# bdwsq1996/Effi-MVS-plus

Hardware: AMD Instinct MI355X
Metric: ref-views/sec (cost-volume hot path: warp + cost volume + 3-D regularisation + cascaded GRU refinement) (higher is better)
Workload: dtype f32 (3x3 MFMA convs: products as 3 bf16 partial products hi*hi+hi*lo+lo*hi, f32 accumulate; all else f32); 1 GPU; cfg3: DTU-shaped 1600x1184, N=5 views (S=4 sources), 3-stage cascade ndepths=48,8,8, GRU iters 3,3,3, seeded-random weights, features of the stock FPN resident in HBM; parallelism=single GPU, views_in_flight=3, arithmetic=split

## Files before the change

### effi_mvs_plus_amd/csrc/api.hip

```cpp
#include "common.hpp"
#include "launch_form.hpp"
#include <cstdlib>
#include <cstring>
#include <mutex>

extern "C" int effi_version(void) { return 200; }

extern "C" const char* effi_error_string(int code) {
    switch (code) {
        case EFFI_OK: return "ok";
        case EFFI_ERR_BADARG: return "bad argument (null pointer, non-positive size, or inconsistent shapes)";
        case EFFI_ERR_UNSUPPORTED: return "shape / channel count not instantiated in this build";
        case EFFI_ERR_LAUNCH: return "kernel launch failed (hipPeekAtLastError)";
        case EFFI_ERR_WORKSPACE: return "no workspace registered for the current device (effi_set_workspace)";
        default: return "unknown error code";
    }
}

static const void* g_workspace[EFFI_MAX_DEVICES];

extern "C" long effi_workspace_bytes(void) { return 256; }

extern "C" int effi_set_workspace(int device, void* workspace, long bytes) {
    if (device < 0 || device >= EFFI_MAX_DEVICES) return EFFI_ERR_BADARG;
// ... 4 lines not shown

extern "C" const void* effi_get_workspace(int device) {
    if (device < 0 || device >= EFFI_MAX_DEVICES) return nullptr;
    return __atomic_load_n(&g_workspace[device], __ATOMIC_ACQUIRE);
}

const float* effi_zero_page() {
    int dev = -1;
    if (hipGetDevice(&dev) != hipSuccess) return nullptr;
    return (const float*)effi_get_workspace(dev);
}

namespace {
const char* const kOptName[EFFI_OPT_COUNT] = {"warp_lds_kb", "dyn_form", "dyn_setup_exact", "dyn_xchg", "pixnet_mfma", "force_mr", "mr4_min",
                                              "mr4_nt2_max", "mr2_min", "wide_tiles", "roll_mr", "roll_zt", "roll_rp", "deconv_mr", "sr_waves", "enc_gen_mr3", "c3_lean", "dyn_win",
                                              "roll_slide"};
long g_opt[EFFI_OPT_COUNT];
std::once_flag g_opt_once;
void load_options() {
    for (int i = 0; i < EFFI_OPT_COUNT; ++i) {
        char env[64] = "EFFI_";
        size_t n = strlen(env);
        for (const char* c = kOptName[i]; *c && n + 1 < sizeof(env); ++c) env[n++] = (*c >= 'a' && *c <= 'z') ? (char)(*c - 32) : *c;
        env[n] = 0;
        const char* v = getenv(env);
        g_opt[i] = (v && *v) ? atol(v) : EFFI_OPT_UNSET;
    }
}
int find_option(const char* name) {
    if (!name) return -1;
    for (int i = 0; i < EFFI_OPT_COUNT; ++i)
// ... 28 lines not shown
    const EffiFormOpts o = effi_form_opts();
    EffiForm f;
    switch (launcher) {
        case EFFI_LF_X3: f = effi_pick_x3(nt, h, w, zb ? planes : 1, zb, sr, o); break;
        case EFFI_LF_X3_BATCH: f = effi_pick_x3_batch(nt, h, w, count, o); break;
        case EFFI_LF_X3_ZB_BATCH: f = effi_pick_x3_zb_batch(nt, h, w, (long)planes * count, o); break;
        case EFFI_LF_X3_PAIR: f = effi_pick_x3_pair(nt, h, w, sr, o); break;
        case EFFI_LF_CONV2D: f = effi_pick_generic(k1 ? 1 : 3, h, w, count); break;
        case EFFI_LF_PLANES3D: f = effi_pick_planes(h, w, (long)planes * count, s2 ? 2 : 4); break;
        case EFFI_LF_K5S2: f = effi_pick_planes(h, w, count, 2); break;
        case EFFI_LF_S2_X3: f = effi_pick_s2_x3(h, w, nt == 1 ? 1 : (nt + 1) / 2, (long)planes * count); break;
        case EFFI_LF_ROLL: f = effi_pick_roll((flags & EFFI_LF_FLAG_OCT2) ? 2 : 1, nt, cout, h, w, planes, count, o); break;
        case EFFI_LF_DECONV_X3: f = effi_pick_deconv_x3(cout, h, w, planes, count, o); break;
        case EFFI_LF_C3_PLANES: f = effi_pick_c3_planes(h, w, planes, count); break;
        case EFFI_LF_DECONV_K3: f = effi_pick_deconv_k3(cout, h, w, planes, count); break;
        default: return EFFI_ERR_BADARG;
    }
    form[0] = f.rows, form[1] = f.cols, form[2] = f.waves, form[3] = f.planes, form[4] = f.variant;
    return EFFI_OK;
}

namespace {
__global__ __launch_bounds__(256) void lds_poison_kernel(unsigned pattern, unsigned* sink) {
    __shared__ unsigned buf[16 * 1024];
    for (int i = threadIdx.x; i < 16 * 1024; i += 256) buf[i] = pattern;
    __syncthreads();
    if (buf[(threadIdx.x * 61) & 16383] != pattern) sink[0] = 1;
}
}

// ... 67 lines not shown
```

### effi_mvs_plus_amd/csrc/common.hpp

```cpp
#pragma once
#include <hip/hip_runtime.h>
#include "../../include/effi_mvs_hip.h"

#define EFFI_LAUNCH_CHECK()                                   \
    do {                                                      \
        if (hipPeekAtLastError() != hipSuccess) return EFFI_ERR_LAUNCH; \
    } while (0)

const float* effi_zero_page();

enum EffiOption {
    EFFI_OPT_WARP_LDS_KB,
    EFFI_OPT_DYN_FORM,
    EFFI_OPT_DYN_SETUP_EXACT,
    EFFI_OPT_DYN_XCHG,
    EFFI_OPT_PIXNET_MFMA,
    EFFI_OPT_FORCE_MR,
    EFFI_OPT_MR4_MIN, EFFI_OPT_MR4_NT2_MAX, EFFI_OPT_MR2_MIN,
    EFFI_OPT_WIDE_TILES,
    EFFI_OPT_ROLL_MR, EFFI_OPT_ROLL_ZT, EFFI_OPT_ROLL_RP,
    EFFI_OPT_DECONV_MR,
    EFFI_OPT_SR_WAVES,
    EFFI_OPT_ENC_GEN_MR3,
    EFFI_OPT_C3_LEAN,
    EFFI_OPT_DYN_WIN,
    EFFI_OPT_ROLL_SLIDE,
    EFFI_OPT_COUNT
};
constexpr long EFFI_OPT_UNSET = -0x7fffffffL;
long effi_option(int id);

static inline hipStream_t effi_s(effi_stream_t s) {
    (void)hipGetLastError();
    return reinterpret_cast<hipStream_t>(s);
}
static inline int effi_cdiv(long a, long b) { return (int)((a + b - 1) / b); }

struct EffiPtrList {
    const float* p[EFFI_MAX_VIEWS + 1];
    const float* const* tbl;
};
// ... 387 lines not shown
```

### effi_mvs_plus_amd/csrc/conv2d_x3.hpp

```cpp
#pragma once
#include "common.hpp"
#include "launch_form.hpp"
#include <type_traits>

#ifdef EFFI_BF16_ONLY
#define EFFI_FN(name) name##_bf16
#else
#define EFFI_FN(name) name
#endif

#ifndef EFFI_ABL
#define EFFI_ABL 0
#endif
#ifndef EFFI_PIPE_FRAGS
#define EFFI_PIPE_FRAGS 0
#endif

#ifndef EFFI_EPI_BATCH
#define EFFI_EPI_BATCH 1
#endif
#ifndef EFFI_EPI_EARLY_MAX
#define EFFI_EPI_EARLY_MAX 16
#endif
#ifndef EFFI_B_EARLY
// ... 23 lines not shown
    const float* aux1;
    const float* disp_range;
    int n_range;
    float* out0;
    float* out1;
    long cstride;
    long ostride;
    int zcount;
    int zin;
    int hin, win;
    const float* zeros;
    const float* xptr0;
    int sr_hp, sr_wp;
    unsigned short* out_sr;
    int aux_q4;
};

struct ConvBatch {
    int n_img;
    long src[EFFI_MAX_SRC];
    long aux0;
    long out0;
};

__device__ __forceinline__ Conv2dArgs conv_batch_image(Conv2dArgs a, const ConvBatch& b, int img) {
#pragma unroll
    for (int i = 0; i < EFFI_MAX_SRC; ++i) a.src[i] += (long)img * b.src[i];
    a.aux0 += (long)img * b.aux0;
    a.out0 += (long)img * b.out0;
    return a;
}

struct EncGenArgs {
    const float* inv_depth; const float* disp_range; int n_range; const float* interval;
    const float* cur_vol; long cds, cps; int Dcur;
    const float* reg_vol; long rds, rps; int Dreg;
    const float* dmin; const float* dmax; long range_ps;
    const float* w_c1; const float* b_c1;
    const float* w_d1; const float* b_d1;
    int hd;
    int off32;
};

__device__ __forceinline__ float apply_act(float v, int act) {
// ... 126 lines not shown

__device__ __forceinline__ void split_octet(const f32x4 (&pa)[8], int px, bf16x8& hi, bf16x8& lo) {
#pragma unroll
    for (int e = 0; e < 8; e += 2) {
        const f32x2 x = {pa[e][px], pa[e + 1][px]};
        const bf16x2 h2 = __builtin_convertvector(x, bf16x2);
        const f32x2 hf = __builtin_convertvector(h2, f32x2);
        const bf16x2 l2 = __builtin_convertvector(x - hf, bf16x2);
        hi[e] = h2[0];
        hi[e + 1] = h2[1];
        lo[e] = l2[0];
        lo[e + 1] = l2[1];
    }
}

template <int NT, int MR, int EPI, bool ZB, bool WIDE, bool SR = false, int NW = 4, bool GEN = false, bool REMAP = true>
__device__ __forceinline__ void conv2d_k3_bf16x3_tile(const Conv2dArgs a, int tiles_x, int ntiles, int bid, int nbid, int bidy,
                                                      const EncGenArgs* gp = nullptr, int gmode = 0) {
    constexpr int NTHR = NW * 64;
    static_assert(!GEN || SR, "generated inputs use the split-resident LDS image");
    static_assert(NW == 4 || (SR && NW == 8), "eight waves: split-resident kernels only");
    constexpr int TR = WIDE ? NW : NW * MR, TW = WIDE ? 16 * MR : 16;
    constexpr int AR = TR + 2, AW = SR ? TW + 2 : TW + 8, AQ = AW / 4, XOFF = SR ? 0 : 3, XLEFT = 4, CCH = 16, NKS = 5;
    constexpr int MROW = WIDE ? 0 : AW * 8, MCOL = WIDE ? 16 * 8 : 0;
    constexpr int APIX = AR * AW, NITEMS = (APIX / 4) * 2;
    constexpr int APIXP = SR ? ((APIX + 15) & ~15) : APIX;
    constexpr int NPART = kHiOnly ? 1 : 2;
    constexpr int NUA = SR ? (NPART * 2 * APIXP + NTHR - 1) / NTHR : 1;
    constexpr int NBF = NKS * NT * 2 * 64;
    constexpr int NB4 = (NBF + NTHR - 1) / NTHR;
    static_assert(SR || NITEMS <= 256, "one staging item per thread");
    static_assert(!(SR && ZB), "split-resident maps are 2-D");
    static_assert(EPI != EFFI_EPI_HEAD && EPI != EFFI_EPI_ADD_UP2, "epilogue not instantiated for the split-precision kernel");
    static_assert((EPI != EFFI_EPI_K1 && EPI != EFFI_EPI_K1UP && EPI != EFFI_EPI_K1HEAD) || !ZB, "the fused 1x1 epilogue is 2-D only");
    constexpr bool kHead = EPI == EFFI_EPI_K1HEAD;
    static_assert(!kHead || (SR && !WIDE && !GEN), "the one-launch depth head reads split-resident maps on 16-column tiles");
// ... 190 lines not shown
                const bf16x4 l4 = __builtin_convertvector(v - __builtin_convertvector(h4, f32x4), bf16x4);
                if (pr < APIX) {
                    const int e = ((lk >> 1) * APIXP + p) * 8 + (lk & 1) * 4;
                    *reinterpret_cast<bf16x4*>(&lds_ah[e]) = h4;
                    if (!kHiOnly) *reinterpret_cast<bf16x4*>(&lds_ah[2 * APIXP * 8 + e]) = l4;
                }
            }
        }
    };

    f32x4 tb[NB4];
    auto fetch_b = [&](int ch) {
#pragma unroll
        for (int j = 0; j < NB4; ++j) {
            const int u = min(tid + j * NTHR, NBF - 1);
            tb[j] = *reinterpret_cast<const f32x4*>(wbf + ((long)ch * NBF + u) * 8);
        }
    };
    constexpr bool kBEarly = SR && !GEN && EFFI_B_EARLY;
    auto stash = [&](int ch) {
        if (!kBEarly || ch == 0) fetch_b(ch);
        if constexpr (GEN) {
            generate(ch);
        } else if constexpr (SR) {
#pragma unroll
            for (int j = 0; j < NUA; ++j) *reinterpret_cast<f32x4*>(&lds_ah[(tid + j * NTHR) * 8]) = pa[j];
        } else if (stager) {
#pragma unroll
            for (int px = 0; px < 4; ++px) {
                bf16x8 hi, lo;
// ... 10 lines not shown
#pragma unroll
    for (int s_ = 0; s_ < NKS; ++s_) {
        const int item = 4 * s_ + lk;
        const int tap = min(item >> 1, 8), oct = item & 1;
        koff[s_] = (((WIDE ? wv : wv * MR) + tap / 3) * AW + li + XOFF + tap % 3 + oct * APIXP) * 8;
    }

    f32x4 acc[MR][NT];
#pragma unroll
    for (int m = 0; m < MR; ++m)
#pragma unroll
        for (int n = 0; n < NT; ++n) acc[m][n] = f32x4{0.0f, 0.0f, 0.0f, 0.0f};

    constexpr bool kBatchT = SR && EFFI_EPI_BATCH != 0 && !(EFFI_ABL & 24) &&
                             (EPI == EFFI_EPI_PLAIN || EPI == EFFI_EPI_GRU_ZR || EPI == EFFI_EPI_GRU_Q);
    constexpr int NZ = (EPI == EFFI_EPI_GRU_ZR) ? NT / 2 : 0;
    constexpr int NH = !kBatchT ? 0 : (EPI == EFFI_EPI_GRU_ZR ? NT - NZ : (EPI == EFFI_EPI_GRU_Q ? NT : 0));
    constexpr int NZQ = (kBatchT && EPI == EFFI_EPI_GRU_Q) ? NT : 0;
    constexpr bool kStateEarly = MR * (NH + NZQ) * 4 <= EFFI_EPI_EARLY_MAX;
    const bool ebatch = kBatchT && (EPI == EFFI_EPI_PLAIN || a.aux_q4);
    f32x4 eb[kBatchT ? NT : 1], eh[MR][NH > 0 ? NH : 1], ez[MR][NZQ > 0 ? NZQ : 1];
    unsigned eqb[MR];
    bool einside[MR];
    auto epi_issue_bias = [&]() {
        if (!ebatch) return;
#pragma unroll
        for (int n = 0; n < NT; ++n) eb[n] = *reinterpret_cast<const f32x4*>(a.bias + n * 16 + 4 * lk);
#pragma unroll
        for (int m = 0; m < MR; ++m) {
            const int x = x0 + li + (WIDE ? 16 * m : 0), y = y0 + (WIDE ? wv : wv * MR + m);
            einside[m] = (y < h) & (x < w);
            eqb[m] = ((unsigned)lk * (unsigned)hw + (einside[m] ? (unsigned)(y * w + x) : 0u)) * 4u;
        }
    };
    auto epi_issue_state = [&]() {
        if (!ebatch) return;
#pragma unroll
        for (int m = 0; m < MR; ++m) {
#pragma unroll
            for (int j = 0; j < NH; ++j) eh[m][j] = *reinterpret_cast<const f32x4*>(a.aux0 + (size_t)(eqb[m] + (unsigned)j * 16u * (unsigned)hw));
#pragma unroll
            for (int j = 0; j < NZQ; ++j) ez[m][j] = *reinterpret_cast<const f32x4*>(a.aux1 + (size_t)(eqb[m] + (unsigned)j * 16u * (unsigned)hw));
        }
    };

    constexpr bool kK1 = (EPI == EFFI_EPI_K1 || EPI == EFFI_EPI_K1UP || kHead) && !(EFFI_ABL & 24) && EFFI_EPI_BATCH != 0;
    f32x4 kb[kK1 ? NT : 1], kex[kK1 ? MR : 1];
    if constexpr (kK1) {
#pragma unroll
        for (int n = 0; n < NT; ++n) kb[n] = *reinterpret_cast<const f32x4*>(a.bias + n * 16 + 4 * lk);
#pragma unroll
// ... 343 lines not shown
                    if (a.act == EFFI_ACT_RELU) {
#pragma unroll
                        for (int r = 0; r < 4; ++r) v[r] = fmaxf(v[r], 0.0f);
                    } else if (a.act != EFFI_ACT_NONE) {
#pragma unroll
                        for (int r = 0; r < 4; ++r) v[r] = apply_act(v[r], a.act);
                    }
                    effi_sr_store4_at(a.out_sr, ub + (unsigned)(4 * n) * plane, lk & 1, v);
                    if (a.out0) {
                        float* dst = a.out0 + (long)(n * 16 + 4 * lk) * a.ostride + (long)y * w + x;
#pragma unroll
                        for (int r = 0; r < 4; ++r) dst[(long)r * a.ostride] = v[r];
                    }
                } else if constexpr (EPI == EFFI_EPI_GRU_ZR) {
                    f32x4 g;
                    if (n < NZ) {
#pragma unroll
                        for (int r = 0; r < 4; ++r) g[r] = effi_sigmoid_split(v[r]) * 1.0f;
                        *reinterpret_cast<f32x4*>(a.out0 + (size_t)(eqb[m] + (unsigned)n * 16u * (unsigned)hw)) = g;
                    } else {
#pragma unroll
                        for (int r = 0; r < 4; ++r) g[r] = effi_sigmoid_split(v[r]) * eh[m][n >= NZ ? n - NZ : 0][r];
                        effi_sr_store4_at(a.out_sr, ub + (unsigned)(4 * (n - NZ)) * plane, lk & 1, g);
                    }
                } else {
                    f32x4 g;
#pragma unroll
                    for (int r = 0; r < 4; ++r) g[r] = (1.0f - ez[m][n][r]) * eh[m][n][r] + ez[m][n][r] * effi_tanh_split(v[r]);
                    *reinterpret_cast<f32x4*>(a.out0 + (size_t)(eqb[m] + (unsigned)n * 16u * (unsigned)hw)) = g;
                    effi_sr_store4_at(a.out_sr, ub + (unsigned)(4 * n) * plane, lk & 1, g);
                }
// ... 11 lines not shown
        for (int n = 0; n < NT; ++n)
            conv_epilogue_store_t<((EPI == EFFI_EPI_K1 || EPI == EFFI_EPI_K1UP || EPI == EFFI_EPI_K1HEAD) ? EFFI_EPI_PLAIN : EPI), SR>(a, acc[m][n], n * 16 + 4 * lk, pix, hw, zpl, y, x,
                                                                                                          kBiasQ ? &gb[n] : nullptr);
    }
}

template <int NT, int MR, int EPI, bool ZB = false, bool WIDE = false, bool SR = false, int NW = 4>
__global__ __launch_bounds__(NW * 64) void conv2d_k3_bf16x3_kernel(const Conv2dArgs a, int tiles_x, int ntiles) {
#ifdef EFFI_STAGGER
    if (SR && gridDim.x > 512) {
        const int slot = (blockIdx.x >> 8) % 3;
        for (int i = 0; i < slot * EFFI_STAGGER; ++i) __builtin_amdgcn_s_sleep(127);
    }
#endif
    conv2d_k3_bf16x3_tile<NT, MR, EPI, ZB, WIDE, SR, NW>(a, tiles_x, ntiles, blockIdx.x, gridDim.x, blockIdx.y);
}

template <int NT, int MR, bool WIDE, bool SR = false, int NW = 4>
__global__ __launch_bounds__(NW * 64) void conv2d_k3_bf16x3_pair_kernel(const Conv2dArgs a0, const Conv2dArgs a1, int tiles_x, int ntiles) {
    if (blockIdx.y == 0) conv2d_k3_bf16x3_tile<NT, MR, EFFI_EPI_PLAIN, false, WIDE, SR, NW>(a0, tiles_x, ntiles, blockIdx.x, gridDim.x, 0);
    else conv2d_k3_bf16x3_tile<NT, MR, EFFI_EPI_PLAIN, false, WIDE, SR, NW>(a1, tiles_x, ntiles, blockIdx.x, gridDim.x, 0);
}

template <int NT, int MR, int EPI, bool WIDE>
__global__ __launch_bounds__(256) void conv2d_k3_bf16x3_batch_kernel(const Conv2dArgs a, const ConvBatch b, int tiles_x, int ntiles) {
    const int t = effi_xcd_remap(blockIdx.y * gridDim.x + blockIdx.x, gridDim.x * gridDim.y);
    const int img = t / ntiles;
    conv2d_k3_bf16x3_tile<NT, MR, EPI, false, WIDE, false, 4, false, false>(conv_batch_image(a, b, img), tiles_x, ntiles, t - img * ntiles,
                                                                           ntiles, 0);
}
// ... 63 lines not shown


template <int NT, int MR>
__global__ __launch_bounds__(256) void conv3d_k3_bf16x3_zb_batch_kernel(const Conv2dArgs a, const ConvBatch b, int tiles_x, int ntiles) {
    conv2d_k3_bf16x3_tile<NT, MR, EFFI_EPI_PLAIN, true, false, false, 4>(conv_batch_image(a, b, blockIdx.z), tiles_x, ntiles, blockIdx.x,
                                                                         gridDim.x, blockIdx.y);
}

template <int NT, int EPI, bool ZB = false, bool SR = false>
static int launch_bf16x3(const Conv2dArgs& a, hipStream_t st, const ConvBatch* bt = nullptr) {
    constexpr bool kShuf = EPI == EFFI_EPI_ADD_SHUF2 || EPI == EFFI_EPI_NHWC_ADD_SHUF2;
    constexpr bool kBatch = !SR && (ZB ? EPI == EFFI_EPI_PLAIN : (EPI == EFFI_EPI_PLAIN || EPI == EFFI_EPI_NHWC || (kShuf && NT <= 2)));
    if (bt && !kBatch) return EFFI_ERR_UNSUPPORTED;
    const EffiFormOpts o = effi_form_opts();
    const long planes = ZB ? a.zcount : 1, n = bt ? bt->n_img : 1;
    const EffiForm f = !bt ? effi_pick_x3(NT, a.h, a.w, planes, ZB, SR, o)
                           : (ZB ? effi_pick_x3_zb_batch(NT, a.h, a.w, planes * n, o) : effi_pick_x3_batch(NT, a.h, a.w, n, o));
    return effi_switch<1, 2, 4>(f.rows, [&](auto MR) {
        return effi_switch<0, 1>(f.variant, [&](auto WIDE) {
            constexpr int mr = MR();
            constexpr bool wide = WIDE() != 0;
            const int tiles_x = effi_cdiv(a.w, wide ? 16 * mr : 16), ntiles = tiles_x * effi_cdiv(a.h, wide ? 4 : 4 * mr);
            if constexpr (kBatch) {
                if (bt) {
                    if constexpr (!ZB)
                        return effi_launch<conv2d_k3_bf16x3_batch_kernel<NT, mr, EPI, wide>>(dim3(ntiles, (unsigned)n), 256, st, a, *bt, tiles_x, ntiles);
                    else if constexpr (!wide)
                        return effi_launch<conv3d_k3_bf16x3_zb_batch_kernel<NT, mr>>(dim3(ntiles, (unsigned)a.zcount, (unsigned)n), 256, st, a, *bt,
                                                                                   tiles_x, ntiles);
                    else
// ... 57 lines not shown
```

### effi_mvs_plus_amd/csrc/conv_host_check.cpp

```cpp
#include "host_check_record.hpp"
#include "conv2d.hip"
#include "conv2d_sr.hip"

namespace {
void show_one(const Conv2dArgs& a) {
    for (int i = 0; i < EFFI_MAX_SRC; ++i) ptr(L("src%d", i).c_str(), a.src[i]);
    for (int i = 0; i < EFFI_MAX_SRC; ++i) if (a.ch[i]) put(" ch%d=%d", i, a.ch[i]);
    FI(a, cin), FI(a, kgroups), FP(a, wpack), FP(a, bias), FI(a, cout), FI(a, h), FI(a, w), FI(a, act), FI(a, hd), FP(a, aux0), FP(a, aux1);
    FP(a, disp_range), FI(a, n_range), FP(a, out0), FP(a, out1), FI(a, cstride), FI(a, ostride), FI(a, zcount), FI(a, zin), FI(a, hin);
    FI(a, win), FP(a, zeros), FP(a, xptr0), FI(a, sr_hp), FI(a, sr_wp), FP(a, out_sr), FI(a, aux_q4);
}
void show_one(const ConvBatch& b) {
    FI(b, n_img);
    for (int i = 0; i < EFFI_MAX_SRC; ++i) if (b.src[i]) put(" src%d=%ld", i, b.src[i]);
    FI(b, aux0), FI(b, out0);
}
void show_one(const EncGenArgs& g) {
    FP(g, inv_depth), FP(g, disp_range), FI(g, n_range), FP(g, interval), FP(g, cur_vol), FI(g, cds), FI(g, cps), FI(g, Dcur), FP(g, reg_vol);
    FI(g, rds), FI(g, rps), FI(g, Dreg), FP(g, dmin), FP(g, dmax), FI(g, range_ps), FP(g, w_c1), FP(g, b_c1), FP(g, w_d1), FP(g, b_d1), FI(g, hd);
    FI(g, off32);
}
void show_one(const DeconvArgs& a) {
    FP(a, in), FP(a, wpack), FP(a, bias), FP(a, skip), FP(a, zeros), FP(a, out), FI(a, cin), FI(a, cout), FI(a, D), FI(a, h), FI(a, w), FI(a, relu);
}
void show_one(const ConvTwiceArgs& a) {
// ... 554 lines not shown
    }
    EXPECT_BADARG(effi_conv2d_k3_bf16x3_pair_f32, S, C8, 2, W, B, O0, S2, C16, 1, W2, B2, O1, 16, 16, 16, 0, nullptr);
    EXPECT_BADARG(effi_conv2d_k3_bf16x3_pair_sr, V, C16, 2, W, B, OS, V2, C32, 1, W2, B2, OS2, 32, 16, 16, hp_of(16), wp_of(16), 0, nullptr);
    EXPECT_BADARG(effi_conv2d_k3_k1_bf16x3_f32, S, C8, 2, W, B, 32, 1, X, 8, W2, B2, 24, 0, 16, 16, O0, nullptr);
    EXPECT_BADARG(effi_conv3d_k3s1_bf16x3_f32, S, C8, 1, W, B, 16, 2, 16, 16, 1, O0, nullptr);
    EXPECT_BADARG(effi_conv3d_k3s1_bf16x3_f32_batch, S, C8, 1, W, B, 16, 2, 16, 16, 1, O0, 2, SS, 0L, nullptr);
    {
        Opt r(EFFI_OPT_ROLL_MR, 3);
        EXPECT_BADARG(effi_conv3d_k3s1_roll_bf16x3_f32, S, C8, 1, W, B, 8, 8, 32, 32, 1, O0, nullptr);
        EXPECT_BADARG(effi_conv3d_k3s1_roll_bf16x3_f32_batch, S, C8, 1, W, B, 16, 8, 32, 32, 1, O0, 2, SS, 0L, nullptr);
    }
    Opt o3(EFFI_OPT_SR_WAVES, 8);
    EXPECT_BADARG(effi_conv2d_k3_bf16x3_pair_sr, V, C16, 2, W, B, OS, V2, C32, 1, W2, B2, OS2, 32, 16, 16, hp_of(16), wp_of(16), 0, nullptr);
}

int main() {
    for (long& v : g_opt) v = EFFI_OPT_UNSET;
#ifndef EFFI_BF16_ONLY
    cases_fp32();
#endif
    std::printf("# split-precision entries: the records of both builds (the second appends _bf16 to the entry names)\n");
    cases_x3();
    cases_sr();
    cases_rows_refused();
    if (g_failures) std::printf("conv host check: %d FAILED\n", g_failures);
    return g_failures ? 1 : 0;
}
```

### effi_mvs_plus_amd/csrc/launch_form.hpp

```cpp
#pragma once
#include "common.hpp"
#include <type_traits>

template <int... Vs, class F>
static int effi_switch_or(int miss, long v, F&& f) {
    int rc = miss;
    (void)(... || (v == Vs ? (rc = f(std::integral_constant<int, Vs>{}), true) : false));
    return rc;
}
template <int... Vs, class F>
static int effi_switch(long v, F&& f) { return effi_switch_or<Vs...>(EFFI_ERR_BADARG, v, f); }
template <int... Vs, class F>
static int effi_switch_nt(long v, F&& f) { return effi_switch_or<Vs...>(EFFI_ERR_UNSUPPORTED, v, f); }

template <auto KERNEL, class... Args>
static int effi_launch(dim3 grid, int threads, hipStream_t st, const Args&... args) {
    hipLaunchKernelGGL(KERNEL, grid, dim3(threads), 0, st, args...);
    return hipPeekAtLastError() == hipSuccess ? EFFI_OK : EFFI_ERR_LAUNCH;
}

#ifndef EFFI_C3_TX
#define EFFI_C3_TX 32
#define EFFI_C3_TY 8
#endif

struct EffiFormOpts {
    long force_mr;
    long mr4_min, mr4_nt2_max, mr2_min;
    long wide_tiles;
    long sr_waves, roll_mr, roll_zt, roll_rp, deconv_mr;
    long roll_slide;
};

static inline long effi_opt_or(int id, long dflt) {
    const long v = effi_option(id);
    return v == EFFI_OPT_UNSET ? dflt : v;
}

static inline EffiFormOpts effi_form_opts() {
    EffiFormOpts o;
    o.force_mr = effi_opt_or(EFFI_OPT_FORCE_MR, 0);
    o.mr4_min = effi_opt_or(EFFI_OPT_MR4_MIN, 400);
    o.mr4_nt2_max = effi_opt_or(EFFI_OPT_MR4_NT2_MAX, 1024);
    o.mr2_min = effi_opt_or(EFFI_OPT_MR2_MIN, 400);
    o.wide_tiles = effi_opt_or(EFFI_OPT_WIDE_TILES, -1);
    o.sr_waves = effi_option(EFFI_OPT_SR_WAVES);
    o.roll_mr = effi_option(EFFI_OPT_ROLL_MR);
    o.roll_zt = effi_option(EFFI_OPT_ROLL_ZT);
    o.roll_rp = effi_option(EFFI_OPT_ROLL_RP);
    o.deconv_mr = effi_option(EFFI_OPT_DECONV_MR);
    o.roll_slide = effi_opt_or(EFFI_OPT_ROLL_SLIDE, 1);
    return o;
}

struct EffiForm {
    int rows;
    int cols;
    int waves;
    int planes;
    int variant;
};

static inline int effi_pick_x3_rows(int nt, int h, int w, long count, const EffiFormOpts& o) {
    const long cols = effi_cdiv(w, 16);
    const long t4 = cols * effi_cdiv(h, 16) * count, t2 = cols * effi_cdiv(h, 8) * count;
    int mr;
    if (t4 >= o.mr4_min && !(nt == 2 && t4 >= o.mr4_nt2_max)) mr = 4;
    else if (t2 >= o.mr2_min) mr = 2;
    else mr = 1;
    if (o.force_mr) mr = (int)o.force_mr;
    return mr;
}

static inline EffiForm effi_pick_x3(int nt, int h, int w, long planes, bool zb, bool sr, const EffiFormOpts& o) {
    const int mr = effi_pick_x3_rows(nt, h, w, planes, o);
    const bool wide = o.wide_tiles >= 0 ? o.wide_tiles != 0 : (mr == 4 && w >= 512 && !zb);
    if (wide) return EffiForm{mr, 16 * mr, 4, 1, 1};
    if (sr && ((o.sr_waves == 8 && mr <= 2) || (o.sr_waves == EFFI_OPT_UNSET && mr == 1 && nt >= 6))) return EffiForm{mr, 16, 8, 1, 0};
    return EffiForm{mr, 16, 4, 1, 0};
}

static inline EffiForm effi_pick_x3_batch(int nt, int h, int w, long n_img, const EffiFormOpts& o) {
    const int mr = effi_pick_x3_rows(nt, h, w, n_img, o);
    const bool wide = o.wide_tiles >= 0 ? o.wide_tiles != 0 : (mr == 4 && w >= 512);
    return wide ? EffiForm{mr, 16 * mr, 4, 1, 1} : EffiForm{mr, 16, 4, 1, 0};
}

static inline EffiForm effi_pick_x3_zb_batch(int nt, int h, int w, long planes, const EffiFormOpts& o) {
    return EffiForm{effi_pick_x3_rows(nt, h, w, planes, o), 16, 4, 1, 0};
}

static inline EffiForm effi_pick_x3_pair(int nt, int h, int w, bool sr, const EffiFormOpts& o) {
    const int mr = effi_pick_x3_rows(nt, h, w, 2, o);
    if (mr == 4 && w >= 512) return EffiForm{4, 64, 4, 1, 1};
// ... 109 lines not shown
```

### effi_mvs_plus_amd/ops.py

```python
from __future__ import annotations

import collections
import ctypes as C
import functools
import os
import threading
from typing import NamedTuple

import weakref

import torch

from . import _lib
from ._lib import EffiLibraryError, check

ACT_NONE, ACT_RELU, ACT_SIGMOID, ACT_TANH = 0, 1, 2, 3
EPI_PLAIN, EPI_GRU_ZR, EPI_GRU_Q, EPI_HEAD, EPI_ADD_UP2, EPI_NHWC = 0, 1, 2, 3, 4, 5
EPI_ADD_SHUF2, EPI_NHWC_ADD_SHUF2 = 9, 10
MAX_VIEWS = 12


class KernelProfile:

    def __init__(self, keys=None):
# ... 46 lines not shown

def uses_split():
    return _PRECISION in ("split", "bf16")


def _x3(name):
    return getattr(_lib.lib(), name + "_bf16" if _PRECISION == "bf16" else name)


_PY_OPTION_DEFAULTS = {"warp_x3": 0, "state_q4": 1, "c1k7_mfma": 1, "k5s2_split": 1, "roll": 1, "conv3d_unaligned_split": 1, "conv3d_s2_split": 1, "fpn_conv0_fused": 1,
                       "fpn_split_head": 1, "csp_pair": 1, "head_taps": 1, "enc_tail": 0, "enc_gen": 1, "reduce_chunk": 2048, "gru_fused": 0, "csp_gen": 0,
                       "head_fused": 1, "head_fused_tile": 0, "clear_fused": 1, "setup_fused": 1, "conf_fused": 1,
                       "fpn_batch": 1}
_PY_OPTS = {k: int(os.environ.get("EFFI_" + k.upper(), v)) for k, v in _PY_OPTION_DEFAULTS.items()}
LIB_OPTIONS = ("warp_lds_kb", "dyn_form", "dyn_setup_exact", "dyn_xchg", "pixnet_mfma", "force_mr", "mr4_min", "mr4_nt2_max", "mr2_min",
               "wide_tiles", "roll_mr", "roll_zt", "roll_rp", "deconv_mr", "sr_waves", "enc_gen_mr3", "c3_lean", "dyn_win", "roll_slide")


def option(name):
    return _PY_OPTS[name]


def get_option(name):
    if name in _PY_OPTS:
        return _PY_OPTS[name]
    if name not in LIB_OPTIONS:
        raise KeyError(name)
    L = _lib.lib()
    v = L.effi_get_option(name.encode())
    return None if v == L.effi_option_unset() else int(v)

# ... 13 lines not shown
    def __init__(self, **kw):
        self.kw, self.before = kw, {}

    def __enter__(self):
        for k, v in self.kw.items():
            self.before[k] = set_option(k, v)
        return self

    def __exit__(self, *exc):
        for k, v in self.before.items():
            set_option(k, v)
        return False


LAUNCHERS = {"x3": 0, "x3_batch": 1, "x3_zb_batch": 2, "x3_pair": 3, "conv2d": 4, "planes3d": 5, "k5s2": 6, "s2_x3": 7, "roll": 8,
             "deconv_x3": 9, "c3_planes": 10, "deconv_k3": 11}
LaunchForm = collections.namedtuple("LaunchForm", "rows cols waves planes variant")


def launch_form(launcher, h, w, nt=1, planes=1, count=1, cout=1, sr=False, zb=False, k1=False, s2=False, oct2=False):
    form = (C.c_int * 5)()
    flags = (1 if sr else 0) | (2 if zb else 0) | (4 if k1 else 0) | (8 if s2 else 0) | (16 if oct2 else 0)
    check(_lib.lib().effi_launch_form(LAUNCHERS[launcher], nt, h, w, planes, count, cout, flags, C.addressof(form)),
          "effi_launch_form")
    return LaunchForm(*form)


def set_profile(p):
    global _PROF
    _PROF = p


def get_profile():
    return _PROF


def _call(key, work, fn, *args):
# ... 2382 lines not shown
```

### include/effi_mvs_hip.h

```cpp
#ifndef EFFI_MVS_HIP_H
#define EFFI_MVS_HIP_H

#ifdef __cplusplus
extern "C" {
#endif

#define EFFI_OK               0
#define EFFI_ERR_BADARG      -1
#define EFFI_ERR_UNSUPPORTED -2
#define EFFI_ERR_LAUNCH      -3
#define EFFI_ERR_WORKSPACE   -4

#define EFFI_MAX_VIEWS 12
#define EFFI_MAX_SRC    3
#define EFFI_VIEW_TABLE_ROW (EFFI_MAX_VIEWS + 2)
#define EFFI_VIEW_TABLE_MAX 64

typedef void* effi_stream_t;

#define EFFI_ACT_NONE    0
#define EFFI_ACT_RELU    1
#define EFFI_ACT_SIGMOID 2
#define EFFI_ACT_TANH    3
#define EFFI_EPI_PLAIN   0
// ... 507 lines not shown
long effi_get_option(const char* name);
long effi_option_unset(void);

enum {
    EFFI_LF_X3 = 0,
    EFFI_LF_X3_BATCH = 1,
    EFFI_LF_X3_ZB_BATCH = 2,
    EFFI_LF_X3_PAIR = 3,
    EFFI_LF_CONV2D = 4,
    EFFI_LF_PLANES3D = 5,
    EFFI_LF_K5S2 = 6,
    EFFI_LF_S2_X3 = 7,
    EFFI_LF_ROLL = 8,
    EFFI_LF_DECONV_X3 = 9,
    EFFI_LF_C3_PLANES = 10,
    EFFI_LF_DECONV_K3 = 11
};
enum { EFFI_LF_FLAG_SR = 1, EFFI_LF_FLAG_ZB = 2, EFFI_LF_FLAG_K1 = 4, EFFI_LF_FLAG_S2 = 8, EFFI_LF_FLAG_OCT2 = 16 };
int effi_launch_form(int launcher, int nt, int h, int w, int planes, int count, int cout, int flags, int* form);

int effi_sr_geometry(int h, int w, int* hp, int* wp);
int effi_sr_clear_border(void* const* maps, const int* planes, const int* h, const int* w, const int* hp, const int* wp, int n_groups,
                         effi_stream_t stream);
int effi_sr_from_planar_f32(const float* in, int channels, int h, int w, void* sr, int hp, int wp, effi_stream_t stream);
int effi_split_tanh_relu_stages_sr_f32(const float* const* ctx, const int* hd, const int* cd, const int* h, const int* w,
                                       float* const* hidden, void* const* hidden_sr, const int* hp, const int* wp, float* const* inp,
                                       const int* hidden_q4, int n_stages, effi_stream_t stream);
int effi_split_tanh_relu_stages_sr_clear_f32(const float* const* ctx, const int* hd, const int* cd, const int* h, const int* w,
                                             float* const* hidden, void* const* hidden_sr, const int* hp, const int* wp,
                                             float* const* inp, const int* hidden_q4, void* const* clear_base, const int* clear_planes,
                                             int n_stages, effi_stream_t stream);
int effi_encoder_inputs_bf16x3_sr(const float* inv_depth, const float* disp_range, int n_range, const float* interval,
                                  const float* cur_vol, long cds, long cps, int Dcur, const float* reg_vol, long rds, long rps,
// ... 64 lines not shown
```

Measured before the change: 629.7 views/s.

## Split split-resident 3x3 GRU convs into N-tile groups across a second grid dimension

Adds a grouped launch form for split-resident bf16x3 3x3 convs. The output N-tiles are partitioned into G groups along blockIdx.y, and each block computes only its group's channels, with weight, bias, output and auxiliary pointers rebased per group. A size-based rule enables 2 or 3 groups for the GRU z|r and q convs at the mid-size (148x200) and large (296x400) cascade stages, aiming to expose more blocks and reduce per-block register and accumulator pressure. In exchange, the input tile is reloaded and reconverted once per group. An sr_ngroups option overrides the rule, and host-side checks cover the picker and the launches.

```diff
diff --git a/effi_mvs_plus_amd/csrc/api.hip b/effi_mvs_plus_amd/csrc/api.hip
--- a/effi_mvs_plus_amd/csrc/api.hip
+++ b/effi_mvs_plus_amd/csrc/api.hip
@@ -42,7 +42,7 @@
 namespace {
 const char* const kOptName[EFFI_OPT_COUNT] = {"warp_lds_kb", "dyn_form", "dyn_setup_exact", "dyn_xchg", "pixnet_mfma", "force_mr", "mr4_min",
                                               "mr4_nt2_max", "mr2_min", "wide_tiles", "roll_mr", "roll_zt", "roll_rp", "deconv_mr", "sr_waves", "enc_gen_mr3", "c3_lean", "dyn_win",
-                                              "roll_slide"};
+                                              "roll_slide", "sr_ngroups"};
 long g_opt[EFFI_OPT_COUNT];
 std::once_flag g_opt_once;
 void load_options() {
@@ -101,6 +101,12 @@
         case EFFI_LF_DECONV_X3: f = effi_pick_deconv_x3(cout, h, w, planes, count, o); break;
         case EFFI_LF_C3_PLANES: f = effi_pick_c3_planes(h, w, planes, count); break;
         case EFFI_LF_DECONV_K3: f = effi_pick_deconv_k3(cout, h, w, planes, count); break;
+        case EFFI_LF_X3_SR: {
+            const int epi = (flags & EFFI_LF_FLAG_ZR) ? EFFI_EPI_GRU_ZR : ((flags & EFFI_LF_FLAG_Q) ? EFFI_EPI_GRU_Q : EFFI_EPI_PLAIN);
+            const int rc = effi_pick_x3_sr(nt, h, w, epi, o, &f);
+            if (rc != EFFI_OK) return rc;
+            break;
+        }
         default: return EFFI_ERR_BADARG;
     }
     form[0] = f.rows, form[1] = f.cols, form[2] = f.waves, form[3] = f.planes, form[4] = f.variant;
diff --git a/effi_mvs_plus_amd/csrc/common.hpp b/effi_mvs_plus_amd/csrc/common.hpp
--- a/effi_mvs_plus_amd/csrc/common.hpp
+++ b/effi_mvs_plus_amd/csrc/common.hpp
@@ -25,6 +25,7 @@
     EFFI_OPT_C3_LEAN,
     EFFI_OPT_DYN_WIN,
     EFFI_OPT_ROLL_SLIDE,
+    EFFI_OPT_SR_NGROUPS,
     EFFI_OPT_COUNT
 };
 constexpr long EFFI_OPT_UNSET = -0x7fffffffL;
diff --git a/effi_mvs_plus_amd/csrc/conv2d_x3.hpp b/effi_mvs_plus_amd/csrc/conv2d_x3.hpp
--- a/effi_mvs_plus_amd/csrc/conv2d_x3.hpp
+++ b/effi_mvs_plus_amd/csrc/conv2d_x3.hpp
@@ -61,6 +61,7 @@
     int sr_hp, sr_wp;
     unsigned short* out_sr;
     int aux_q4;
+    int nt_all;
 };
 
 struct ConvBatch {
@@ -75,6 +76,33 @@
     for (int i = 0; i < EFFI_MAX_SRC; ++i) a.src[i] += (long)img * b.src[i];
     a.aux0 += (long)img * b.aux0;
     a.out0 += (long)img * b.out0;
+    return a;
+}
+
+template <int NT, int EPI>
+__device__ __forceinline__ Conv2dArgs conv_group_args(Conv2dArgs a, int g) {
+    const int nb = g * NT;
+    const long hw = (long)a.h * a.w, plane8 = (long)a.sr_hp * a.sr_wp * 8;
+    a.wpack += (long)nb * 128 * 4;
+    a.bias += nb * 16;
+    if (EPI == EFFI_EPI_GRU_ZR) {
+        const int rb = nb - a.nt_all / 2;
+        if (rb < 0) {
+            a.out0 += (long)nb * 16 * hw;
+            a.hd = NT * 16;
+        } else {
+            a.aux0 += (long)rb * 16 * hw;
+            a.out_sr += (long)rb * 4 * plane8;
+            a.hd = 0;
+        }
+    } else {
+        if (EPI == EFFI_EPI_GRU_Q) {
+            a.aux0 += (long)nb * 16 * hw;
+            a.aux1 += (long)nb * 16 * hw;
+        }
+        if (a.out0) a.out0 += (long)nb * 16 * hw;
+        a.out_sr += (long)nb * 4 * plane8;
+    }
     return a;
 }
 
@@ -231,12 +259,14 @@
     }
 }
 
-template <int NT, int MR, int EPI, bool ZB, bool WIDE, bool SR = false, int NW = 4, bool GEN = false, bool REMAP = true>
+template <int NT, int MR, int EPI, bool ZB, bool WIDE, bool SR = false, int NW = 4, bool GEN = false, bool REMAP = true, bool GRP = false>
 __device__ __forceinline__ void conv2d_k3_bf16x3_tile(const Conv2dArgs a, int tiles_x, int ntiles, int bid, int nbid, int bidy,
                                                       const EncGenArgs* gp = nullptr, int gmode = 0) {
     constexpr int NTHR = NW * 64;
     static_assert(!GEN || SR, "generated inputs use the split-resident LDS image");
     static_assert(NW == 4 || (SR && NW == 8), "eight waves: split-resident kernels only");
+    static_assert(!GRP || (SR && !GEN && !WIDE && NW == 4 && (EPI == EFFI_EPI_PLAIN || EPI == EFFI_EPI_GRU_ZR || EPI == EFFI_EPI_GRU_Q)),
+                  "N-tile groups: the four-wave split-resident plain / GRU forms");
     constexpr int TR = WIDE ? NW : NW * MR, TW = WIDE ? 16 * MR : 16;
     constexpr int AR = TR + 2, AW = SR ? TW + 2 : TW + 8, AQ = AW / 4, XOFF = SR ? 0 : 3, XLEFT = 4, CCH = 16, NKS = 5;
     constexpr int MROW = WIDE ? 0 : AW * 8, MCOL = WIDE ? 16 * 8 : 0;
@@ -457,6 +487,11 @@
 #pragma unroll
         for (int j = 0; j < NB4; ++j) {
             const int u = min(tid + j * NTHR, NBF - 1);
+            if constexpr (GRP) {
+                const int ks = u / (NT * 128), r_ = u - ks * (NT * 128);
+                tb[j] = *reinterpret_cast<const f32x4*>(wbf + (((long)ch * NKS + ks) * (a.nt_all * 128) + r_) * 8);
+                continue;
+            }
             tb[j] = *reinterpret_cast<const f32x4*>(wbf + ((long)ch * NBF + u) * 8);
         }
     };
@@ -497,7 +532,8 @@
 
     constexpr bool kBatchT = SR && EFFI_EPI_BATCH != 0 && !(EFFI_ABL & 24) &&
                              (EPI == EFFI_EPI_PLAIN || EPI == EFFI_EPI_GRU_ZR || EPI == EFFI_EPI_GRU_Q);
-    constexpr int NZ = (EPI == EFFI_EPI_GRU_ZR) ? NT / 2 : 0;
+    constexpr int NZ = (EPI == EFFI_EPI_GRU_ZR && !GRP) ? NT / 2 : 0;
+    const bool zgrp = GRP && EPI == EFFI_EPI_GRU_ZR && a.hd != 0;
     constexpr int NH = !kBatchT ? 0 : (EPI == EFFI_EPI_GRU_ZR ? NT - NZ : (EPI == EFFI_EPI_GRU_Q ? NT : 0));
     constexpr int NZQ = (kBatchT && EPI == EFFI_EPI_GRU_Q) ? NT : 0;
     constexpr bool kStateEarly = MR * (NH + NZQ) * 4 <= EFFI_EPI_EARLY_MAX;
@@ -517,7 +553,7 @@
         }
     };
     auto epi_issue_state = [&]() {
-        if (!ebatch) return;
+        if (!ebatch || zgrp) return;
 #pragma unroll
         for (int m = 0; m < MR; ++m) {
 #pragma unroll
@@ -891,7 +927,7 @@
                     }
                 } else if constexpr (EPI == EFFI_EPI_GRU_ZR) {
                     f32x4 g;
-                    if (n < NZ) {
+                    if (GRP ? zgrp : n < NZ) {
 #pragma unroll
                         for (int r = 0; r < 4; ++r) g[r] = effi_sigmoid_split(v[r]) * 1.0f;
                         *reinterpret_cast<f32x4*>(a.out0 + (size_t)(eqb[m] + (unsigned)n * 16u * (unsigned)hw)) = g;
@@ -933,6 +969,12 @@
     }
 #endif
     conv2d_k3_bf16x3_tile<NT, MR, EPI, ZB, WIDE, SR, NW>(a, tiles_x, ntiles, blockIdx.x, gridDim.x, blockIdx.y);
+}
+
+template <int NT, int MR, int EPI>
+__global__ __launch_bounds__(256) void conv2d_k3_bf16x3_group_kernel(const Conv2dArgs a, int tiles_x, int ntiles) {
+    conv2d_k3_bf16x3_tile<NT, MR, EPI, false, false, true, 4, false, true, true>(conv_group_args<NT, EPI>(a, blockIdx.y), tiles_x, ntiles, blockIdx.x,
+                                                                                gridDim.x, 0);
 }
 
 template <int NT, int MR, bool WIDE, bool SR = false, int NW = 4>
@@ -1026,6 +1068,24 @@
     if (bt && !kBatch) return EFFI_ERR_UNSUPPORTED;
     const EffiFormOpts o = effi_form_opts();
     const long planes = ZB ? a.zcount : 1, n = bt ? bt->n_img : 1;
+    if constexpr (SR && (EPI == EFFI_EPI_PLAIN || EPI == EFFI_EPI_GRU_ZR || EPI == EFFI_EPI_GRU_Q)) {
+        EffiForm fg;
+        const int rc = effi_pick_x3_sr(NT, a.h, a.w, EPI, o, &fg);
+        if (rc != EFFI_OK) return rc;
+        if (fg.planes > 1)
+            return effi_switch<2, 3, 4, 6>(fg.planes, [&](auto G) {
+                if constexpr (NT % G() == 0 && (EPI != EFFI_EPI_GRU_ZR || G() % 2 == 0)) {
+                    return effi_switch<1, 2, 4>(fg.rows, [&](auto MR) {
+                        Conv2dArgs ag = a;
+                        ag.nt_all = NT;
+                        const int tiles_x = effi_cdiv(a.w, 16), ntiles = tiles_x * effi_cdiv(a.h, 4 * MR());
+                        return effi_launch<conv2d_k3_bf16x3_group_kernel<NT / G(), MR(), EPI>>(dim3(ntiles, G()), 256, st, ag, tiles_x, ntiles);
+                    });
+                } else {
+                    return (int)EFFI_ERR_BADARG;
+                }
+            });
+    }
     const EffiForm f = !bt ? effi_pick_x3(NT, a.h, a.w, planes, ZB, SR, o)
                            : (ZB ? effi_pick_x3_zb_batch(NT, a.h, a.w, planes * n, o) : effi_pick_x3_batch(NT, a.h, a.w, n, o));
     return effi_switch<1, 2, 4>(f.rows, [&](auto MR) {
diff --git a/effi_mvs_plus_amd/csrc/conv_host_check.cpp b/effi_mvs_plus_amd/csrc/conv_host_check.cpp
--- a/effi_mvs_plus_amd/csrc/conv_host_check.cpp
+++ b/effi_mvs_plus_amd/csrc/conv_host_check.cpp
@@ -8,7 +8,7 @@
     for (int i = 0; i < EFFI_MAX_SRC; ++i) if (a.ch[i]) put(" ch%d=%d", i, a.ch[i]);
     FI(a, cin), FI(a, kgroups), FP(a, wpack), FP(a, bias), FI(a, cout), FI(a, h), FI(a, w), FI(a, act), FI(a, hd), FP(a, aux0), FP(a, aux1);
     FP(a, disp_range), FI(a, n_range), FP(a, out0), FP(a, out1), FI(a, cstride), FI(a, ostride), FI(a, zcount), FI(a, zin), FI(a, hin);
-    FI(a, win), FP(a, zeros), FP(a, xptr0), FI(a, sr_hp), FI(a, sr_wp), FP(a, out_sr), FI(a, aux_q4);
+    FI(a, win), FP(a, zeros), FP(a, xptr0), FI(a, sr_hp), FI(a, sr_wp), FP(a, out_sr), FI(a, aux_q4), FI(a, nt_all);
 }
 void show_one(const ConvBatch& b) {
     FI(b, n_img);
@@ -593,6 +593,72 @@
     EXPECT_BADARG(effi_conv2d_k3_bf16x3_pair_sr, V, C16, 2, W, B, OS, V2, C32, 1, W2, B2, OS2, 32, 16, 16, hp_of(16), wp_of(16), 0, nullptr);
 }
 
+static void cases_sr_groups() {
+    void* const OS = P<void>(50);
+    auto fail = [&](const std::string& what) { std::printf("FAILED: sr groups: %s\n", what.c_str()); ++g_failures; };
+    auto pick = [&](int nt, int h, int w, int epi, EffiForm* f) { return effi_pick_x3_sr(nt, h, w, epi, effi_form_opts(), f); };
+    const struct { int epi, nt, h, w; EffiForm want; } layers[] = {
+        {EFFI_EPI_GRU_ZR, 6, 148, 200, {2, 16, 4, 2, 0}}, {EFFI_EPI_GRU_Q, 3, 148, 200, {2, 16, 4, 3, 0}},
+        {EFFI_EPI_GRU_ZR, 4, 296, 400, {4, 16, 4, 1, 0}}, {EFFI_EPI_GRU_Q, 2, 296, 400, {4, 16, 4, 2, 0}},
+        {EFFI_EPI_GRU_ZR, 2, 592, 800, {2, 16, 4, 1, 0}}, {EFFI_EPI_GRU_Q, 1, 592, 800, {4, 64, 4, 1, 1}}};
+    for (const auto& l : layers) {
+        EffiForm f{}, f1{};
+        const EffiForm& w_ = l.want;
+        if (pick(l.nt, l.h, l.w, l.epi, &f) != EFFI_OK || f.rows != w_.rows || f.cols != w_.cols || f.waves != w_.waves || f.planes != w_.planes ||
+            f.variant != w_.variant)
+            fail(L("rule: epilogue %d, %d N-tiles at %dx%d -> rows %d cols %d waves %d groups %d variant %d", l.epi, l.nt, l.h, l.w, f.rows, f.cols,
+                   f.waves, f.planes, f.variant));
+        Opt o(EFFI_OPT_SR_NGROUPS, 1);
+        const EffiForm x = effi_pick_x3(l.nt, l.h, l.w, 1, false, true, effi_form_opts());
+        if (pick(l.nt, l.h, l.w, l.epi, &f1) != EFFI_OK || f1.rows != x.rows || f1.cols != x.cols || f1.waves != x.waves || f1.planes != 1 ||
+            f1.variant != x.variant)
+            fail(L("sr_ngroups = 1 is not the form of effi_pick_x3: %d N-tiles at %dx%d", l.nt, l.h, l.w));
+    }
+    for (int nt : {1, 2, 3, 4, 6})
+        for (int epi : {EFFI_EPI_PLAIN, EFFI_EPI_GRU_ZR, EFFI_EPI_GRU_Q}) {
+            EffiForm f{};
+            if (epi == EFFI_EPI_GRU_ZR && (nt & 1)) continue;
+            if (pick(nt, 592, 800, epi, &f) != EFFI_OK || f.planes != 1) fail(L("592x800 takes groups: epilogue %d, %d N-tiles", epi, nt));
+            if (pick(nt, 74, 100, epi, &f) != EFFI_OK || f.planes != 1) fail(L("74x100 takes groups: epilogue %d, %d N-tiles", epi, nt));
+        }
+    for (int epi : {EFFI_EPI_PLAIN, EFFI_EPI_GRU_ZR, EFFI_EPI_GRU_Q})
+        for (int nt : {1, 2, 3, 4, 6})
+            for (long g : {0L, 2L, 3L, 4L, 5L, 6L, 8L}) {
+                if (epi == EFFI_EPI_GRU_ZR && (nt & 1)) continue;
+                Opt o(EFFI_OPT_SR_NGROUPS, g);
+                EffiForm f{};
+                const bool legal = (g == 2 || g == 3 || g == 4 || g == 6) && nt % g == 0 && (epi != EFFI_EPI_GRU_ZR || g % 2 == 0);
+                const int rc = pick(nt, 74, 100, epi, &f);
+                if (legal ? (rc != EFFI_OK || f.planes != g || f.waves != 4 || f.cols != 16 || f.variant != 0) : rc != EFFI_ERR_BADARG)
+                    fail(L("forced %ld groups, epilogue %d, %d N-tiles -> %s", g, epi, nt, rc_name(rc)));
+            }
+    auto has = [&](const char* what) { return g_rec.find(what) != std::string::npos; };
+    g_rec.clear();
+    int rc = EFFI_FN(effi_conv2d_k3_bf16x3_sr)(V, C16, 2, W, B, 96, 148, 200, hp_of(148), wp_of(200), EFFI_EPI_GRU_ZR | EFFI_EPI_Q4, 0, A0, A1, O0, OS, nullptr);
+    if (rc != EFFI_OK || !has("conv2d_k3_bf16x3_group_kernel<3, 2, 1> grid 247,2,1 block 256") || !has(" nt_all=6")) fail("z | r launch at 148x200:" + g_rec);
+    g_rec.clear();
+    rc = EFFI_FN(effi_conv2d_k3_bf16x3_sr)(V, C16, 3, W, B, 48, 148, 200, hp_of(148), wp_of(200), EFFI_EPI_GRU_Q | EFFI_EPI_Q4, 0, A0, A1, O0, OS, nullptr);
+    if (rc != EFFI_OK || !has("conv2d_k3_bf16x3_group_kernel<1, 2, 2> grid 247,3,1 block 256") || !has(" nt_all=3")) fail("q launch at 148x200:" + g_rec);
+    {
+        Opt o(EFFI_OPT_SR_NGROUPS, 2), o2(EFFI_OPT_FORCE_MR, 4);
+        g_rec.clear();
+        rc = EFFI_FN(effi_conv2d_k3_bf16x3_sr)(V, C16, 2, W, B, 32, 74, 100, hp_of(74), wp_of(100), EFFI_EPI_PLAIN, EFFI_ACT_RELU, A0, A1, nullptr, OS, nullptr);
+        if (rc != EFFI_OK || !has("conv2d_k3_bf16x3_group_kernel<1, 4, 0> grid 35,2,1 block 256") || !has(" nt_all=2")) fail("forced plain launch:" + g_rec);
+        g_rec.clear();
+        rc = EFFI_FN(effi_conv2d_k3_k1_bf16x3_sr)(V, C16, 2, W, B, 32, 1, X, 8, W2, B2, 32, 0, 74, 100, hp_of(74), wp_of(100), O0, nullptr, nullptr);
+        if (rc != EFFI_OK || has("group_kernel") || has("nt_all")) fail("fused-1x1 launch with sr_ngroups = 2:" + g_rec);
+    }
+    {
+        Opt o(EFFI_OPT_SR_NGROUPS, 3);
+        EXPECT_BADARG(effi_conv2d_k3_bf16x3_sr, V, C16, 2, W, B, 96, 74, 100, hp_of(74), wp_of(100), EFFI_EPI_GRU_ZR, 0, A0, A1, O0, OS, nullptr);
+        EXPECT_BADARG(effi_conv2d_k3_bf16x3_sr, V, C16, 2, W, B, 32, 74, 100, hp_of(74), wp_of(100), EFFI_EPI_GRU_Q, 0, A0, A1, O0, OS, nullptr);
+    }
+    {
+        Opt o(EFFI_OPT_SR_NGROUPS, 2), o2(EFFI_OPT_WIDE_TILES, 1);
+        EXPECT_BADARG(effi_conv2d_k3_bf16x3_sr, V, C16, 2, W, B, 32, 74, 100, hp_of(74), wp_of(512), EFFI_EPI_PLAIN, 0, A0, A1, O0, OS, nullptr);
+    }
+}
+
 int main() {
     for (long& v : g_opt) v = EFFI_OPT_UNSET;
 #ifndef EFFI_BF16_ONLY
@@ -602,6 +668,7 @@
     cases_x3();
     cases_sr();
     cases_rows_refused();
+    cases_sr_groups();
     if (g_failures) std::printf("conv host check: %d FAILED\n", g_failures);
     return g_failures ? 1 : 0;
 }
diff --git a/effi_mvs_plus_amd/csrc/launch_form.hpp b/effi_mvs_plus_amd/csrc/launch_form.hpp
--- a/effi_mvs_plus_amd/csrc/launch_form.hpp
+++ b/effi_mvs_plus_amd/csrc/launch_form.hpp
@@ -30,6 +30,7 @@
     long wide_tiles;
     long sr_waves, roll_mr, roll_zt, roll_rp, deconv_mr;
     long roll_slide;
+    long sr_ngroups;
 };
 
 static inline long effi_opt_or(int id, long dflt) {
@@ -50,6 +51,7 @@
     o.roll_rp = effi_option(EFFI_OPT_ROLL_RP);
     o.deconv_mr = effi_option(EFFI_OPT_DECONV_MR);
     o.roll_slide = effi_opt_or(EFFI_OPT_ROLL_SLIDE, 1);
+    o.sr_ngroups = effi_option(EFFI_OPT_SR_NGROUPS);
     return o;
 }
 
@@ -78,6 +80,30 @@
     if (wide) return EffiForm{mr, 16 * mr, 4, 1, 1};
     if (sr && ((o.sr_waves == 8 && mr <= 2) || (o.sr_waves == EFFI_OPT_UNSET && mr == 1 && nt >= 6))) return EffiForm{mr, 16, 8, 1, 0};
     return EffiForm{mr, 16, 4, 1, 0};
+}
+
+struct EffiSrGroups { int groups, rows; };
+static inline EffiSrGroups effi_sr_groups_rule(int nt, int h, int w, int epi, const EffiFormOpts& o) {
+    const long t = (long)effi_cdiv(w, 16) * effi_cdiv(h, 4);
+    const bool mid = t >= 400 && t < 1024, large = t >= 1024 && t < 4096;
+    if (epi == EFFI_EPI_GRU_ZR && mid && nt == 6 && o.sr_waves != 8) return {2, 2};
+    if (epi == EFFI_EPI_GRU_ZR && mid && nt == 4) return {2, 2};
+    if (epi == EFFI_EPI_GRU_Q && mid && nt == 3) return {3, 2};
+    if (epi == EFFI_EPI_GRU_Q && large && nt == 2) return {2, 4};
+    return {1, 0};
+}
+static inline int effi_pick_x3_sr(int nt, int h, int w, int epi, const EffiFormOpts& o, EffiForm* f) {
+    *f = effi_pick_x3(nt, h, w, 1, false, true, o);
+    const bool ruled = o.sr_ngroups == EFFI_OPT_UNSET;
+    const EffiSrGroups r = ruled ? (o.wide_tiles > 0 ? EffiSrGroups{1, 0} : effi_sr_groups_rule(nt, h, w, epi, o)) : EffiSrGroups{(int)o.sr_ngroups, 0};
+    const int g = r.groups;
+    if (g == 1) return EFFI_OK;
+    if ((g != 2 && g != 3 && g != 4 && g != 6) || nt % g != 0 || (epi == EFFI_EPI_GRU_ZR && g % 2 != 0)) return EFFI_ERR_BADARG;
+    if (epi != EFFI_EPI_PLAIN && epi != EFFI_EPI_GRU_ZR && epi != EFFI_EPI_GRU_Q) return EFFI_ERR_BADARG;
+    if (o.wide_tiles > 0) return EFFI_ERR_BADARG;
+    const int rows = (r.rows && !o.force_mr) ? r.rows : effi_pick_x3_rows(nt / g, h, w, g, o);
+    *f = EffiForm{rows, 16, 4, g, 0};
+    return EFFI_OK;
 }
 
 static inline EffiForm effi_pick_x3_batch(int nt, int h, int w, long n_img, const EffiFormOpts& o) {
diff --git a/effi_mvs_plus_amd/ops.py b/effi_mvs_plus_amd/ops.py
--- a/effi_mvs_plus_amd/ops.py
+++ b/effi_mvs_plus_amd/ops.py
@@ -84,7 +84,8 @@
                        "fpn_batch": 1}
 _PY_OPTS = {k: int(os.environ.get("EFFI_" + k.upper(), v)) for k, v in _PY_OPTION_DEFAULTS.items()}
 LIB_OPTIONS = ("warp_lds_kb", "dyn_form", "dyn_setup_exact", "dyn_xchg", "pixnet_mfma", "force_mr", "mr4_min", "mr4_nt2_max", "mr2_min",
-               "wide_tiles", "roll_mr", "roll_zt", "roll_rp", "deconv_mr", "sr_waves", "enc_gen_mr3", "c3_lean", "dyn_win", "roll_slide")
+               "wide_tiles", "roll_mr", "roll_zt", "roll_rp", "deconv_mr", "sr_waves", "enc_gen_mr3", "c3_lean", "dyn_win", "roll_slide",
+               "sr_ngroups")
 
 
 def option(name):
@@ -128,13 +129,13 @@
 
 
 LAUNCHERS = {"x3": 0, "x3_batch": 1, "x3_zb_batch": 2, "x3_pair": 3, "conv2d": 4, "planes3d": 5, "k5s2": 6, "s2_x3": 7, "roll": 8,
-             "deconv_x3": 9, "c3_planes": 10, "deconv_k3": 11}
+             "deconv_x3": 9, "c3_planes": 10, "deconv_k3": 11, "x3_sr": 12}
 LaunchForm = collections.namedtuple("LaunchForm", "rows cols waves planes variant")
 
 
-def launch_form(launcher, h, w, nt=1, planes=1, count=1, cout=1, sr=False, zb=False, k1=False, s2=False, oct2=False):
+def launch_form(launcher, h, w, nt=1, planes=1, count=1, cout=1, sr=False, zb=False, k1=False, s2=False, oct2=False, zr=False, q=False):
     form = (C.c_int * 5)()
-    flags = (1 if sr else 0) | (2 if zb else 0) | (4 if k1 else 0) | (8 if s2 else 0) | (16 if oct2 else 0)
+    flags = (1 if sr else 0) | (2 if zb else 0) | (4 if k1 else 0) | (8 if s2 else 0) | (16 if oct2 else 0) | (32 if zr else 0) | (64 if q else 0)
     check(_lib.lib().effi_launch_form(LAUNCHERS[launcher], nt, h, w, planes, count, cout, flags, C.addressof(form)),
           "effi_launch_form")
     return LaunchForm(*form)
diff --git a/include/effi_mvs_hip.h b/include/effi_mvs_hip.h
--- a/include/effi_mvs_hip.h
+++ b/include/effi_mvs_hip.h
@@ -545,9 +545,11 @@
     EFFI_LF_ROLL = 8,
     EFFI_LF_DECONV_X3 = 9,
     EFFI_LF_C3_PLANES = 10,
-    EFFI_LF_DECONV_K3 = 11
+    EFFI_LF_DECONV_K3 = 11,
+    EFFI_LF_X3_SR = 12
 };
-enum { EFFI_LF_FLAG_SR = 1, EFFI_LF_FLAG_ZB = 2, EFFI_LF_FLAG_K1 = 4, EFFI_LF_FLAG_S2 = 8, EFFI_LF_FLAG_OCT2 = 16 };
+enum { EFFI_LF_FLAG_SR = 1, EFFI_LF_FLAG_ZB = 2, EFFI_LF_FLAG_K1 = 4, EFFI_LF_FLAG_S2 = 8, EFFI_LF_FLAG_OCT2 = 16, EFFI_LF_FLAG_ZR = 32,
+       EFFI_LF_FLAG_Q = 64 };
 int effi_launch_form(int launcher, int nt, int h, int w, int planes, int count, int cout, int flags, int* form);
 
 int effi_sr_geometry(int h, int w, int* hp, int* wp);
```

After: 631.0 views/s, median of 5. Within noise of the previous version (+0.2%).
